# Sweetroll97/GaussianProcessPathModelling

Measured on AMD Instinct MI355X. Metric: gp_fit_predict_points_per_sec, higher is better.
Workload: dtype f64; 1 GPU; C3: exact GP fit+predict, N=65536 d=3 rbf float64, M=4096, inputs resident in HBM; N=65536, d=3, M=4096, kernel=rbf, block=2048, parallelism=1 gpu

## Files before the change

gaussianprocesspathmodelling_amd/csrc/gpx_api.hip:

```cpp
#include <hip/hip_runtime.h>
#include <dlfcn.h>

#include <algorithm>
#include <climits>
#include <cmath>
#include <cstdio>
#include <cstdlib>
#include <cstring>
#include <functional>
#include <new>
#include <string>
#include <vector>

#include "../../include/gpx.h"
#include "gpx_cov.h"
#include "gpx_env.h"
#include "gpx_internal.h"

using namespace gpx;

namespace {

thread_local std::string g_create_error;

// ... 150 lines not shown
}

bool bad_mem_kind(int32_t mem_kind) { return !(mem_kind == GPX_MEM_HOST || mem_kind == GPX_MEM_DEVICE); }

int fetch_ids(gpx_handle* h, const int32_t* src, int64_t n, int32_t mem_kind, std::vector<int32_t>& out) {
  out.resize((size_t)n);
  if (mem_kind == GPX_MEM_HOST) {
    std::copy(src, src + n, out.begin());
    return GPX_OK;
  }
  if (!h->group) HIPCHK(h, hipSetDevice(h->cfg.device));
  HIPCHK(h, hipMemcpy(out.data(), src, (size_t)n * sizeof(int32_t), hipMemcpyDefault));
  return GPX_OK;
}

int64_t first_below_minus_one(const int32_t* ids, int64_t n) {
  return std::find_if(ids, ids + n, [](int32_t v) { return v < -1; }) - ids;
}

bool variance_ok(double v) { return v >= 0.0 && std::isfinite(v); }
bool path_ls_ok(const double* ls_path, int32_t n) {
  return std::all_of(ls_path, ls_path + n, [](double l) { return l > 0.0 && std::isfinite(l); });
}

#define MATERN12_NO_GRAD "Matern-1/2 is not differentiable (its sample paths have no derivative)"
#define NOT_TWICE_DIFFERENTIABLE \
  "the kernel is not twice differentiable (only RBF and Matern-5/2 sample paths have a second derivative)"
#define HESS_D_LIMIT "second derivatives are built for at most 8 input dimensions (d > 8)"

#define LAUNCHCHK(h)                                                                                  \
  do {                                                                                                \
    if (take_launch_error())                                                                          \
      return fail(h, GPX_E_ARG, "internal error: a triangular-solve operand was not 128-byte aligned"); \
  } while (0)

int ensure(gpx_handle* h, DevBuf& b, size_t bytes) {
  if (b.cap >= bytes && b.p) return GPX_OK;
  if (b.p) HIPCHK(h, hipFree(b.p));
  b.p = nullptr;
  b.cap = 0;
  HIPCHK(h, hipMalloc(&b.p, bytes));
  b.cap = bytes;
  return GPX_OK;
}

hipEvent_t next_event(gpx_handle* h) {
  if (h->ev_used == h->ev_pool.size()) {
    hipEvent_t e;
    if (hipEventCreate(&e) != hipSuccess) return nullptr;
    h->ev_pool.push_back(e);
  }
  return h->ev_pool[h->ev_used++];
}

int record_event(gpx_handle* h, hipStream_t a, const char* site, hipEvent_t* e) {
  if (!(*e = next_event(h))) {
    char msg[64];
    snprintf(msg, sizeof msg, "hipEventCreate failed (%s)", site);
    return fail(h, GPX_E_HIP, msg);
  }
  HIPCHK(h, hipEventRecord(*e, a));
  return GPX_OK;
}

int stream_waits(gpx_handle* h, hipStream_t b, hipStream_t a, const char* site) {
  hipEvent_t e;
  if (int rc = record_event(h, a, site, &e)) return rc;
  HIPCHK(h, hipStreamWaitEvent(b, e, 0));
  return GPX_OK;
}

struct Roctx {
  int (*push)(const char*) = nullptr;
  int (*pop)() = nullptr;
};
const Roctx& roctx() {
  static const Roctx r = [] {
    Roctx x;
    EnvKnobs env;
    env_read(env, EnvAt::process);
    if (!env.roctx) return x;
    void* lib = nullptr;
    for (const char* n : {"librocprofiler-sdk-roctx.so.1", "librocprofiler-sdk-roctx.so", "libroctx64.so.4", "libroctx64.so"})
      if ((lib = dlopen(n, RTLD_NOW | RTLD_NOLOAD))) break;
    if (!lib)
      for (const char* n : {"librocprofiler-sdk-roctx.so.1", "librocprofiler-sdk-roctx.so"})
        if ((lib = dlopen(n, RTLD_NOW | RTLD_LOCAL))) break;
    if (!lib) return x;
    x.push = reinterpret_cast<int (*)(const char*)>(dlsym(lib, "roctxRangePushA"));
    x.pop = reinterpret_cast<int (*)()>(dlsym(lib, "roctxRangePop"));
    if (!x.push || !x.pop) x.push = nullptr, x.pop = nullptr;
    return x;
  }();
  return r;
}

const char* phase_name(const gpx_handle* h, const double* t) {
  const gpx_timings& tm = h->tm;
#define GPX_PHASE(f) \
  if (t == &tm.f) return "gpx:" #f;
  GPX_PHASE(h2d) GPX_PHASE(kbuild) GPX_PHASE(chol) GPX_PHASE(solve) GPX_PHASE(logdet) GPX_PHASE(fit_total)
  GPX_PHASE(kstar) GPX_PHASE(mean) GPX_PHASE(trsm) GPX_PHASE(var) GPX_PHASE(d2h) GPX_PHASE(predict_total)
  GPX_PHASE(comm) GPX_PHASE(chol_diag) GPX_PHASE(chol_trsm) GPX_PHASE(chol_strip) GPX_PHASE(chol_syrk)
  GPX_PHASE(grad_trtri) GPX_PHASE(grad_trace) GPX_PHASE(grad_total) GPX_PHASE(refine)
#undef GPX_PHASE
  return "gpx:phase";
}

struct PhaseScope {
  gpx_handle* h;
  Phase ph;
  bool on;
  hipStream_t s;
  bool ranged = false;
  PhaseScope(gpx_handle* h_, double* target, bool enable = true, hipStream_t stream = nullptr)
      : h(h_), on(enable), s(stream ? stream : h_->st) {
    if (roctx().push) ranged = roctx().push(phase_name(h, target)) >= 0;
    if (!on) return;
    ph.a = next_event(h);
    ph.b = next_event(h);
    ph.target = target;
    if (ph.a) (void)hipEventRecord(ph.a, s);
  }
  ~PhaseScope() {
    if (ranged) (void)roctx().pop();
    if (!on) return;
    if (ph.b) (void)hipEventRecord(ph.b, s);
    if (ph.a && ph.b) h->phases.push_back(ph);
  }
};

void collect_phases(gpx_handle* h) {
  for (auto& p : h->phases) {
    float ms = 0.f;
    if (hipEventElapsedTime(&ms, p.a, p.b) == hipSuccess) *p.target += ms;
  }
  h->phases.clear();
  h->ev_used = 0;
}


int flag_handover_probe(gpx_handle* h) {
  if (h->flag_ok >= 0) return GPX_OK;
  if (h->env.chain_flag >= 0) return GPX_OK;
  if (h->env.counters_collected || !h->st3) {
    h->flag_ok = 0;
    return GPX_OK;
  }
  unsigned* d = nullptr;
  unsigned seen = 0;
  HIPCHK(h, hipMalloc(&d, 64));
  hipError_t e = hipMemsetAsync(d, 0, 64, h->st);
  if (e == hipSuccess) e = hipStreamSynchronize(h->st);
  if (e == hipSuccess) {
    launch_flag_probe_wait(d, d + 1, 1u << 15, h->st3);
    launch_flag_probe_set(d, h->st);
    e = hipStreamSynchronize(h->st3);
  }
  if (e == hipSuccess) e = hipStreamSynchronize(h->st);
  if (e == hipSuccess) e = hipMemcpy(&seen, d + 1, sizeof(unsigned), hipMemcpyDeviceToHost);
  (void)hipFree(d);
  HIPCHK(h, e);
  h->flag_ok = seen ? 1 : 0;
  return GPX_OK;
}

bool chain_flag_enabled(const gpx_handle* h) {
  if (h->env.chain_flag >= 0) return h->env.chain_flag != 0;
  return !h->env.counters_collected && h->flag_ok == 1;
}

bool fused_strip_in_force(const gpx_handle* h) { return h->env.fused_strip && chain_flag_enabled(h); }
bool split_strip_in_force(const gpx_handle* h) { return h->env.split_strip && !fused_strip_in_force(h); }

bool retry_with_events(gpx_handle* h, bool retried) {
  if (retried || h->env.chain_flag >= 0) return false;
  h->flag_ok = 0;
  h->flag_retries += 1;
  return true;
}

struct LatencyGuard {
  ~LatencyGuard() { set_latency_mode(0); }
};
struct ReserveGuard {
  ~ReserveGuard() { reserve_ring(nullptr, 0); }
};
constexpr int RESV_RING = 1024;


template <typename T>
struct InvWork {
  T* W = nullptr;
  T* U = nullptr;
  int64_t ldu = 0;
  int nbw = 0;
  hipStream_t aux = nullptr;
  hipEvent_t ready = nullptr;
  hipEvent_t copied[2] = {};
  unsigned seq = 0;
};

template <typename T>
int diag_enqueue(gpx_handle* h, T* A, int64_t ld, int64_t o, int nbp, T* Winv, int* info, int64_t gidx0,
                 hipStream_t s, InvWork<T>* iw = nullptr) {
  T* Wp = nullptr;
  unsigned* dflag = reinterpret_cast<unsigned*>(info + 9);
  unsigned seq = iw ? iw->seq : 0;
  const bool use_flag = chain_flag_enabled(h);
  if (iw) {
    Wp = iw->W + (o / iw->nbw) * (int64_t)iw->nbw * iw->nbw;
    hipEvent_t e0 = next_event(h);
    if (!e0) return fail(h, GPX_E_HIP, "hipEventCreate failed (block inverse)");
    if (seq == 0) HIPCHK(h, hipMemsetAsync(dflag, 0, sizeof(unsigned), s));
    HIPCHK(h, hipEventRecord(e0, s));
    HIPCHK(h, hipStreamWaitEvent(iw->aux, e0, 0));
    HIPCHK(h, hipMemsetAsync(iw->U, 0, (size_t)iw->nbw * iw->ldu * sizeof(T), iw->aux));
    launch_set_diag_one_t<T>(iw->U, iw->ldu, nbp, iw->aux);
    HIPCHK(h, hipMemsetAsync(Wp, 0, (size_t)iw->nbw * iw->nbw * sizeof(T), iw->aux));
  }
  const int diag_step = h->env.diag_step;
  const int nq = nbp / KB;
  for (int q = 0; q < nq;) {
    const int w = (diag_step == 128 && q + 1 < nq) ? 2 : 1;
    const int64_t oq = o + (int64_t)q * KB;
    T* Aqq = A + oq * ld + oq;
    T* Wq = Winv + (oq / KB) * (KB * KB);
    seq += 2;
    if (w == 2)
      launch_potf2_128<T>(Aqq, ld, Wq, gidx0 + oq, info, s, iw && use_flag ? dflag : nullptr, seq);
    else
      launch_potf2_64<T>(Aqq, ld, Wq, gidx0 + oq, info, s, iw && use_flag ? dflag : nullptr, seq);
    const int64_t rem = o + nbp - (oq + w * KB);
    if (rem > 0) {
      T* panel = A + (oq + w * KB) * ld + oq;
      launch_trsm_rlt<T>(panel, ld, rem, Aqq, ld, Wq, w * KB, nullptr, 0, s);
      launch_gemm_nt<T>(64, A + (oq + w * KB) * ld + (oq + w * KB), ld, panel, ld, panel, ld, rem, rem, w * KB, 1, 0, s);
    }
    if (iw) {
      if (use_flag) {
        if (q > 0) {
          launch_wait_counter(dflag, seq - 1, info, iw->aux);
          launch_inv_extend<T>(iw->U, iw->ldu, A + o * ld + o, ld, Winv + (o / KB) * (KB * KB), q, q + w, Wp,
                               iw->nbw, iw->aux, 1);
        }
        launch_wait_counter(dflag, seq, info, iw->aux);
      } else {
        if (int rc = stream_waits(h, iw->aux, s, "block inverse")) return rc;
        launch_inv_extend<T>(iw->U, iw->ldu, A + o * ld + o, ld, Winv + (o / KB) * (KB * KB), q, q + w, Wp, iw->nbw,
                             iw->aux, 1);
      }
      launch_inv_extend<T>(iw->U, iw->ldu, A + o * ld + o, ld, Winv + (o / KB) * (KB * KB), q, q + w, Wp, iw->nbw,
                           iw->aux, 2);
    }
    q += w;
  }
  if (iw) {
    iw->seq = seq;
    if (int rc = record_event(h, iw->aux, "block inverse", &iw->ready)) return rc;
  }
  return GPX_OK;
}

template <typename T>
int panel_solve_enqueue(gpx_handle* h, T* A, int64_t ld, int64_t o, int nbp, int64_t rows_main, int64_t nx,
                        const T* Winv, T* P, int64_t ldp, hipStream_t s, InvWork<T>* iw, int set, int64_t row0 = 0,
                        hipEvent_t prev = nullptr, bool last = true) {
  T* Apanel = A + (o + nbp + row0) * ld + o;
  P += row0 * ldp;
  const int64_t rows = rows_main + nx;
  if (rows <= 0) {
    if (iw && last && row0 > 0) {
      if (int rc = record_event(h, h->st4, "panel copy", &iw->copied[set])) return rc;
    }
    return GPX_OK;
  }
  if (!iw) {
    launch_trsm_rlt<T>(Apanel, ld, rows, A + o * ld + o, ld, Winv + (o / KB) * (KB * KB), nbp, P, ldp, s);
    return GPX_OK;
  }
  const T* Wp = iw->W + (o / iw->nbw) * (int64_t)iw->nbw * iw->nbw;
  HIPCHK(h, hipStreamWaitEvent(s, iw->ready, 0));
  if (row0 == 0 && last) prev = iw->copied[set];
  if (prev) HIPCHK(h, hipStreamWaitEvent(s, prev, 0));
  const int tile_main = gemm_nt_tile((rows_main % 128 == 0 && nbp % 128 == 0) ? 128 : 64, rows_main, nbp, 4);
  if (rows_main > 0 && nx > 0 && tile_main == 64) {
    launch_gemm_nt_fixed<T>(64, P, ldp, Apanel, ld, Wp, iw->nbw, rows, nbp, nbp, 4, 1, s);
  } else {
    if (rows_main > 0) launch_gemm_nt_fixed<T>(tile_main, P, ldp, Apanel, ld, Wp, iw->nbw, rows_main, nbp, nbp, 4, 1, s);
    if (nx > 0)
      launch_gemm_nt<T>(64, P + rows_main * ldp, ldp, Apanel + rows_main * ld, ld, Wp, iw->nbw, nx, nbp, nbp, 4, 1,
                        s);
  }
  if (int rc = stream_waits(h, h->st4, s, "panel copy")) return rc;
  launch_copy2d<T>(Apanel, ld, P, ldp, rows, nbp, h->st4);
  if (last) return record_event(h, h->st4, "panel copy", &iw->copied[set]);
  return GPX_OK;
}

inline int64_t split_rows_128(int64_t nr, int64_t nc) {
  return (nr > 128 && nr % 128 != 0 && nc % 128 == 0) ? nr / 128 * 128 : nr;
}

template <typename T>
int chol_enqueue(gpx_handle* h, T* A, int64_t ld, int64_t n, int nb, T* Winv, T* P0, T* P1,
                 int64_t ldp, int* info, int64_t gidx0, bool profile, int64_t nx = 0,
                 InvWork<T>* iw = nullptr, int64_t nx_side = 0, int rest_split_arg = -1) {
  hipStream_t s0 = h->st, s1 = h->st2;
  T* Pbuf[2] = {P0, P1};
  int rc;
  const EnvKnobs& env = h->env;
  const bool fuse_env = fused_strip_in_force(h);
  unsigned* ctr = reinterpret_cast<unsigned*>(info + 8);
  unsigned target = 0;
  auto is_fused = [&](int64_t o) -> bool {
    if (!fuse_env || o >= n) return false;
    const int nbp = (int)std::min<int64_t>(nb, n - o);
    const int64_t ntrail = n - (o + nbp);
    if (ntrail <= 0) return false;
    const int nbn = (int)std::min<int64_t>(nb, ntrail);
    const int64_t nrest = ntrail - nbn;
    if (nrest <= 0 || ntrail % 128 != 0 || nbn % 128 != 0) return false;
    return gemm_nt_tile(128, nrest, nrest, 1) == 128 && gemm_nt_tile(128, ntrail, nbn, 2) == 128;
  };
  auto bordered_update = [&](int64_t o, const T* Pc, hipStream_t s) {
    const int nbp = (int)std::min<int64_t>(nb, n - o);
    const int64_t t0 = o + nbp, ntrail = n - t0;
    if (nx <= 0 || ntrail <= 0) return;
    launch_gemm_nt<T>(nx % 128 == 0 && ntrail % 128 == 0 ? 128 : 64, A + n * ld + t0, ld, Pc + ntrail * ldp, ldp, Pc,
                      ldp, nx, ntrail, nbp, 0, 0, s);
  };
  auto bordered_block = [&](int64_t o, const T* Pc, hipStream_t s, int64_t c0, int64_t nc, int64_t r0, int64_t nr) {
    const int nbp = (int)std::min<int64_t>(nb, n - o);
    const int64_t t0 = o + nbp, ntrail = n - t0;
    if (nr <= 0 || nc <= 0) return;
    const int64_t na = split_rows_128(nr, nc);
    launch_gemm_nt<T>(na % 128 == 0 && nc % 128 == 0 ? 128 : 64, A + (n + r0) * ld + c0, ld, Pc + (ntrail + r0) * ldp, ldp,
                      Pc + (c0 - t0) * ldp, ldp, na, nc, nbp, 0, 0, s);
    if (na < nr)
      launch_gemm_nt<T>(64, A + (n + r0 + na) * ld + c0, ld, Pc + (ntrail + r0 + na) * ldp, ldp, Pc + (c0 - t0) * ldp, ldp,
                        nr - na, nc, nbp, 0, 0, s);
  };
  auto update_is_big = [&](int64_t o) -> bool {
    if (o >= n) return false;
    const int nbp = (int)std::min<int64_t>(nb, n - o);
    const int64_t ntrail = n - (o + nbp);
    if (ntrail <= 0) return false;
    const int nbn = (int)std::min<int64_t>(nb, ntrail);
    const int64_t nrest = ntrail - nbn;
    return nrest > 0 && ntrail % 128 == 0 && nbn % 128 == 0 && gemm_nt_tile(128, nrest, nrest, 1) == 128;
  };
  const bool split_env = split_strip_in_force(h);
  const bool top_env = env.solve_top;
  const int rest_split = rest_split_arg >= 0 ? rest_split_arg : env.rest_split;
  const int64_t nxs = split_env ? nx_side : 0, nxc = nx - nxs;
  auto side_solve = [&](int64_t o, T* Pp, hipStream_t s) -> int {
    if (nxs <= 0) return GPX_OK;
    const int nbp = (int)std::min<int64_t>(nb, n - o);
    T* Aside = A + (n + nxc) * ld + o;
    T* Pside = Pp + ((n - o - nbp) + nxc) * ldp;
    if (!iw) {
      launch_trsm_rlt<T>(Aside, ld, nxs, A + o * ld + o, ld, Winv + (o / KB) * (KB * KB), nbp, Pside, ldp, s);
      return GPX_OK;
    }
    HIPCHK(h, hipStreamWaitEvent(s, iw->ready, 0));
    const T* Wp = iw->W + (o / iw->nbw) * (int64_t)iw->nbw * iw->nbw;
    const int64_t na = split_rows_128(nxs, nbp);
    launch_gemm_nt<T>(na % 128 == 0 && nbp % 128 == 0 ? 128 : 64, Pside, ldp, Aside, ld, Wp, iw->nbw, na, nbp, nbp, 4, 1, s);
    if (na < nxs) launch_gemm_nt<T>(64, Pside + na * ldp, ldp, Aside + na * ld, ld, Wp, iw->nbw, nxs - na, nbp, nbp, 4, 1, s);
    launch_copy2d<T>(Aside, ld, Pside, ldp, nxs, nbp, s);
    return GPX_OK;
  };
  LatencyGuard latency_guard;
  set_latency_mode(1);
  const int resv_k = env.cu_self_reserve;
  ReserveGuard reserve_guard;
  if (resv_k > 0 && split_env) {
    if ((rc = ensure(h, h->resv_ring, (size_t)RESV_RING * 8 * sizeof(unsigned)))) return rc;
    HIPCHK(h, hipMemsetAsync(h->resv_ring.p, 0, (size_t)RESV_RING * 8 * sizeof(unsigned), s0));
    reserve_ring((unsigned*)h->resv_ring.p, RESV_RING, env.resv_form);
  }
  const bool any_fused = is_fused(0);
  if (any_fused) HIPCHK(h, hipMemsetAsync(ctr, 0, sizeof(unsigned), s0));
  {
    const int nb0 = (int)std::min<int64_t>(nb, n);
    {
      PhaseScope ps(h, &h->tm.chol_diag, profile);
      if ((rc = diag_enqueue(h, A, ld, 0, nb0, Winv, info, gidx0, s0, iw))) return rc;
    }
    {
      PhaseScope ps(h, &h->tm.chol_trsm, profile);
      if ((rc = panel_solve_enqueue(h, A, ld, 0, nb0, n - nb0, nxc, Winv, Pbuf[0], ldp, s0, iw, 0))) return rc;
    }
    if (any_fused) {
      bordered_update(0, Pbuf[0], s0);
      if ((rc = stream_waits(h, s1, s0, "look-ahead"))) return rc;
    }
  }
  hipEvent_t e_main = nullptr;
  if (split_env && n > nb && (rc = record_event(h, s0, "look-ahead", &e_main))) return rc;
  int step = 0;
  for (int64_t o = 0; o < n; o += nb, ++step) {
    const int nbp = (int)std::min<int64_t>(nb, n - o);
    const int64_t t0 = o + nbp;
    const int64_t ntrail = n - t0;
    if (ntrail <= 0) {
      if ((rc = side_solve(o, Pbuf[step & 1], s0))) return rc;
      break;
    }
    T* Pc = Pbuf[step & 1];
    T* Pn = Pbuf[(step + 1) & 1];
    const int nbn = (int)std::min<int64_t>(nb, ntrail);
    const int64_t nrest = ntrail - nbn;
    const int tile = (ntrail % 128 == 0 && nbn % 128 == 0) ? 128 : 64;
    hipEvent_t e_panel = next_event(h);
    if (!e_panel) return fail(h, GPX_E_HIP, "hipEventCreate failed (look-ahead)");
    set_latency_mode(update_is_big(o) ? 0 : 1);
    if (is_fused(o)) {
      {
        PhaseScope ps(h, &h->tm.chol_syrk, profile);
        target += launch_gemm_nt_fused<T>(A + t0 * ld + t0, ld, Pc, ldp, ntrail, nbn, nbp, ctr, s0);
        h->tm.syrk_flops += (double)ntrail * (double)(ntrail + 1) * (double)nbp;
        h->tm.syrk_launches += 1;
      }
      launch_wait_counter(ctr, target, info, s1);
      {
        PhaseScope ps(h, &h->tm.chol_diag, profile, s1);
        if ((rc = diag_enqueue(h, A, ld, t0, nbn, Winv, info, gidx0, s1, iw))) return rc;
      }
      {
        PhaseScope ps(h, &h->tm.chol_trsm, profile, s1);
        if ((rc = panel_solve_enqueue(h, A, ld, t0, nbn, nrest, nx, Winv, Pn, ldp, s1, iw, (step + 1) & 1))) return rc;
      }
      HIPCHK(h, hipEventRecord(e_panel, s1));
      if (is_fused(t0)) bordered_update(t0, Pn, s1);
      HIPCHK(h, hipStreamWaitEvent(s0, e_panel, 0));
      continue;
    }
    if (split_env) {
      hipStream_t sm = s0;
      const int resv_it = (resv_k > 0 && (env.resv_all || ntrail <= (int64_t)(rest_split + 1) * nb)) ? resv_k : 0;
      if (e_main) HIPCHK(h, hipStreamWaitEvent(s1, e_main, 0));
      {
        PhaseScope ps(h, &h->tm.chol_strip, profile, s1);
        launch_gemm_nt<T>(tile, A + t0 * ld + t0, ld, Pc, ldp, Pc, ldp, nbn, nbn, nbp, 1, 0, s1);
      }
      set_reserve_mode(resv_it);
      {
        PhaseScope ps(h, &h->tm.chol_strip, profile, sm);
        if (nrest > 0)
          launch_gemm_nt<T>(tile, A + (t0 + nbn) * ld + t0, ld, Pc + (int64_t)nbn * ldp, ldp, Pc, ldp, nrest, nbn, nbp, 0,
                            0, sm);
        bordered_block(o, Pc, sm, t0, nbn, 0, nxc);
      }
      hipEvent_t e_below;
      if ((rc = record_event(h, sm, "look-ahead", &e_below))) return rc;
      const int nbn2 = (int)std::min<int64_t>(nb, nrest);
      const bool ahead = nrest > nbn2 && nrest <= (int64_t)rest_split * nb;
      T* Cr = A + (t0 + nbn) * ld + (t0 + nbn);
      const T* Pr = Pc + (int64_t)nbn * ldp;
      if (ahead) {
        {
          PhaseScope ps(h, &h->tm.chol_strip, profile, sm);
          launch_gemm_nt<T>(tile, Cr, ld, Pr, ldp, Pr, ldp, nrest, nbn2, nbp, 2, 0, sm);
        }
        if ((rc = record_event(h, sm, "look-ahead", &e_main))) return rc;
      }
      const int64_t nr = ahead ? nrest - nbn2 : nrest, off = ahead ? nbn2 : 0;
      if (nr > 0) {
        const bool big = gemm_nt_tile(tile, nr, nr, 1) == 128;
        PhaseScope ps(h, big ? &h->tm.chol_syrk : &h->tm.chol_strip, profile, sm);
        launch_gemm_nt<T>(tile, Cr + off * ld + off, ld, Pr + off * ldp, ldp, Pr + off * ldp, ldp, nr, nr, nbp, 1, 0, sm);
        if (big) {
          h->tm.syrk_flops += (double)nr * (double)(nr + 1) * (double)nbp;
          h->tm.syrk_launches += 1;
        }
      }
      if (!ahead && (rc = record_event(h, sm, "look-ahead", &e_main))) return rc;
      {
        PhaseScope ps(h, &h->tm.chol_strip, profile, sm);
        bordered_block(o, Pc, sm, t0 + nbn, nrest, 0, nxc);
        if ((rc = side_solve(o, Pc, sm))) return rc;
        bordered_block(o, Pc, sm, t0, ntrail, nxc, nxs);
      }
      set_reserve_mode(0);
      {
        PhaseScope ps(h, &h->tm.chol_diag, profile, s1);
        set_reserve_chain(resv_it > 0 ? env.resv_chain : 0);
        rc = diag_enqueue(h, A, ld, t0, nbn, Winv, info, gidx0, s1, iw);
        set_reserve_chain(0);
        if (rc) return rc;
      }
      HIPCHK(h, hipStreamWaitEvent(s1, e_below, 0));
      const int64_t top = (iw && top_env) ? std::min<int64_t>(nrest, nb) : nrest;
      hipEvent_t prev_copied = iw ? iw->copied[(step + 1) & 1] : nullptr;
      {
        PhaseScope ps(h, &h->tm.chol_trsm, profile, s1);
        if (top < nrest || (iw && top_env)) {
          if ((rc = panel_solve_enqueue(h, A, ld, t0, nbn, top, 0, Winv, Pn, ldp, s1, iw, (step + 1) & 1, 0, prev_copied,
                                        false)))
            return rc;
        } else if ((rc = panel_solve_enqueue(h, A, ld, t0, nbn, nrest, nxc, Winv, Pn, ldp, s1, iw, (step + 1) & 1))) {
          return rc;
        }
      }
      HIPCHK(h, hipEventRecord(e_panel, s1));
      HIPCHK(h, hipStreamWaitEvent(sm, e_panel, 0));
      if (top < nrest || (iw && top_env)) {
        PhaseScope ps(h, &h->tm.chol_trsm, profile, sm);
        set_reserve_mode(resv_it);
        rc = panel_solve_enqueue(h, A, ld, t0, nbn, nrest - top, nxc, Winv, Pn, ldp, sm, iw, (step + 1) & 1, top, prev_copied,
                                 true);
        set_reserve_mode(0);
        if (rc) return rc;
      }
      continue;
    }
    {
      PhaseScope ps(h, &h->tm.chol_strip, profile);
      set_latency_mode(1);
      launch_gemm_nt<T>(tile, A + t0 * ld + t0, ld, Pc, ldp, Pc, ldp, ntrail, nbn, nbp, 2, 0, s0);
      set_latency_mode(update_is_big(o) ? 0 : 1);
      bordered_update(o, Pc, s0);
    }
    if ((rc = stream_waits(h, s1, s0, "look-ahead"))) return rc;
    {
      {
        PhaseScope ps(h, &h->tm.chol_diag, profile, s1);
        if ((rc = diag_enqueue(h, A, ld, t0, nbn, Winv, info, gidx0, s1, iw))) return rc;
      }
      {
        PhaseScope ps(h, &h->tm.chol_trsm, profile, s1);
        if ((rc = panel_solve_enqueue(h, A, ld, t0, nbn, nrest, nx, Winv, Pn, ldp, s1, iw, (step + 1) & 1))) return rc;
      }
    }
    HIPCHK(h, hipEventRecord(e_panel, s1));
    if (nrest > 0) {
      const bool big = gemm_nt_tile(tile, nrest, nrest, 1) == 128;
      PhaseScope ps(h, big ? &h->tm.chol_syrk : &h->tm.chol_strip, profile);
      launch_gemm_nt<T>(tile, A + (t0 + nbn) * ld + (t0 + nbn), ld, Pc + (int64_t)nbn * ldp, ldp,
                        Pc + (int64_t)nbn * ldp, ldp, nrest, nrest, nbp, 1, 0, s0);
      if (big) {
        h->tm.syrk_flops += (double)nrest * (double)(nrest + 1) * (double)nbp;
        h->tm.syrk_launches += 1;
      }
    }
    HIPCHK(h, hipStreamWaitEvent(s0, e_panel, 0));
  }
  if (iw) {
    for (hipStream_t sj : {iw->aux, h->st4})
      if ((rc = stream_waits(h, s0, sj, "join"))) return rc;
  }
  return GPX_OK;
}

template <typename T>
int chol_two_level_enqueue(gpx_handle* h, T* A, int64_t ld, int64_t n, int nb, T* Winv, T* P0, T* P1, int64_t ldp,
                           int* info, int64_t gidx0, bool profile, int64_t nx = 0, InvWork<T>* iw = nullptr,
                           int64_t nx_side = 0) {
  const EnvKnobs& env = h->env;
  const int64_t c = std::max<int64_t>(1, (n / 2 + nb / 2) / nb) * nb, np = n - c;
  const int64_t smin = env.strassen_min;
  const int depth = smin > 0 ? (env.strassen_diag ? 2 : 1) : 0;
  const int64_t hh = np / 2 / 128 * 128, ldt = c / 2 + ld_skew<T>();
  const bool fits = P1 > P0 && strassen_temp_elems(np - hh, hh, c, ld_skew<T>()) <= 2 * (size_t)(P1 - P0);
  const bool wanted = depth == 0 || (fits && (sizeof(T) == 8 || env.strassen_f32));
  if (env.two_level_from <= 0 || n < env.two_level_from || !iw || nx_side != 0 || np < 256 || n % 128 != 0 || nb % 128 != 0 ||
      (nx != 0 && nx != RHS_ROWS) || !wanted)
    return chol_enqueue<T>(h, A, ld, n, nb, Winv, P0, P1, ldp, info, gidx0, profile, nx, iw, nx_side);
  int rc;
  hipStream_t s0 = h->st, s1 = h->st2;
  T *TA = P0, *TB = nullptr;
  const int rs = env.rest_split / 2;
  if ((rc = chol_enqueue<T>(h, A, ld, c, nb, Winv, P0, P1, ldp, info, gidx0, profile, np + nx, iw, np + nx, rs))) return rc;
  T* A22 = A + c * ld + c;
  const T* L21 = A + c * ld;
  hipEvent_t e_rows = nullptr;
  if (nx > 0) {
    if ((rc = stream_waits(h, s1, s0, "deep update"))) return rc;
    PhaseScope ps(h, &h->tm.chol_strip, profile, s1);
    launch_gemm_nt<T>(64, A + n * ld + c, ld, A + n * ld, ld, L21, ld, nx, np, c, 0, 0, s1);
    if ((rc = record_event(h, s1, "deep update", &e_rows))) return rc;
  }
  {
    PhaseScope ps(h, &h->tm.chol_syrk, profile);
    std::function<void(int64_t, int64_t, int)> deep = [&](int64_t o, int64_t sz, int lv) {
      const int64_t s1z = sz / 2 / 128 * 128, s2z = sz - s1z;
      if (lv <= 0 || s1z < 256 || std::min(s1z, s2z) / 256 * 128 < smin) {
        launch_gemm_nt<T>(128, A22 + o * ld + o, ld, L21 + o * ld, ld, L21 + o * ld, ld, sz, sz, c, 1, 0, s0);
        h->tm.syrk_flops += (double)sz * (double)(sz + 1) * (double)c;
        h->tm.syrk_launches += 1;
        return;
      }
      deep(o, s1z, lv - 1);
      TB = TA + (s2z / 256 * 128) * ldt;
      h->tm.syrk_flops += strassen_nt<T>(A22 + (o + s1z) * ld + o, ld, L21 + (o + s1z) * ld, ld, L21 + o * ld, ld, s2z, s1z,
                                         c, TA, TB, ldt, s0);
      h->tm.syrk_launches += 7;
      deep(o + s1z, s2z, lv - 1);
    };
    deep(0, np, depth);
  }
  if (e_rows) HIPCHK(h, hipStreamWaitEvent(s0, e_rows, 0));
  InvWork<T> iw2;
  iw2.W = iw->W + (c / iw->nbw) * (int64_t)iw->nbw * iw->nbw;
  iw2.U = iw->U;
  iw2.ldu = iw->ldu;
  iw2.nbw = iw->nbw;
  iw2.aux = iw->aux;
  rc = chol_enqueue<T>(h, A22, ld, np, nb, Winv + (c / KB) * (KB * KB), P0, P0 + (np + nx) * ldp, ldp, info, gidx0 + c, profile,
                       nx, &iw2, 0, rs);
  iw->seq = iw2.seq;
  return rc;
}

template <typename T>
struct SolveWork {
  const T* W = nullptr;
  int nbw = 0;
  T *T0 = nullptr, *T1 = nullptr;
  int64_t ldt = 0;
};

template <typename T>
int solve_fwd_enqueue(gpx_handle* h, T* XT, int64_t rows, const T* L, int64_t ld, int64_t n, int nb,
                      const T* Winv, const SolveWork<T>* wb = nullptr) {
  hipStream_t s0 = h->st, s1 = h->st2;
  const int tile = (rows % 128 == 0) ? 128 : 64;
  LatencyGuard latency_guard;
  set_latency_mode(1);
  if (rows < 128 || !s1) {
    for (int64_t o = 0; o < n; o += nb) {
      const int nbp = (int)std::min<int64_t>(nb, n - o);
      launch_trsm_rlt<T>(XT + o, ld, rows, L + o * ld + o, ld, Winv + (o / KB) * (KB * KB), nbp, nullptr,
                         0, s0);
      const int64_t ntrail = n - (o + nbp);
      if (ntrail > 0)
        launch_gemm_nt<T>((ntrail % 128 == 0) ? tile : 64, XT + o + nbp, ld, XT + o, ld,
                          L + (o + nbp) * ld + o, ld, rows, ntrail, nbp, 0, 0, s0);
    }
    return GPX_OK;
  }
  const bool dense = wb && wb->nbw == nb && wb->T0 && h->st4;
  T* Ts[2] = {dense ? wb->T0 : nullptr, dense ? wb->T1 : nullptr};
  hipEvent_t e_copy[2] = {nullptr, nullptr};
  const int64_t ldt = dense ? wb->ldt : 0;
  auto block_solve = [&](int64_t o, int nbp, int set, hipStream_t s) -> int {
    if (!dense) {
      launch_trsm_rlt<T>(XT + o, ld, rows, L + o * ld + o, ld, Winv + (o / KB) * (KB * KB), nbp, nullptr, 0, s);
      return GPX_OK;
    }
    if (e_copy[set]) HIPCHK(h, hipStreamWaitEvent(s, e_copy[set], 0));
    launch_gemm_nt<T>((rows % 128 == 0 && nbp % 128 == 0) ? 128 : 64, Ts[set], ldt, XT + o, ld,
                      wb->W + (o / nb) * (int64_t)nb * nb, nb, rows, nbp, nbp, 4, 1, s);
    hipEvent_t e = next_event(h);
    e_copy[set] = next_event(h);
    if (!e || !e_copy[set]) return fail(h, GPX_E_HIP, "hipEventCreate failed (block solve)");
    HIPCHK(h, hipEventRecord(e, s));
    HIPCHK(h, hipStreamWaitEvent(h->st4, e, 0));
    launch_copy2d<T>(XT + o, ld, Ts[set], ldt, rows, nbp, h->st4);
    HIPCHK(h, hipEventRecord(e_copy[set], h->st4));
    return GPX_OK;
  };
  int rc;
  if ((rc = block_solve(0, (int)std::min<int64_t>(nb, n), 0, s0))) return rc;
  int step = 0;
  for (int64_t o = 0; o < n; o += nb, ++step) {
    const int nbp = (int)std::min<int64_t>(nb, n - o);
    const int64_t t0 = o + nbp, ntrail = n - t0;
    if (ntrail <= 0) break;
    const int nbn = (int)std::min<int64_t>(nb, ntrail);
    const int64_t nrest = ntrail - nbn;
    const int tl = (nbn % 128 == 0 && nrest % 128 == 0) ? tile : 64;
    const int cur = step & 1;
    const T* Ablk = dense ? Ts[cur] : XT + o;
    const int64_t lda = dense ? ldt : ld;
    set_latency_mode(1);
    launch_gemm_nt<T>(tl, XT + t0, ld, Ablk, lda, L + t0 * ld + o, ld, rows, nbn, nbp, 0, 0, s0);
    set_latency_mode(nrest > 0 && gemm_nt_tile(tl, rows, nrest, 0) == 128 ? 0 : 1);
    hipEvent_t e_strip = next_event(h), e_panel = next_event(h);
    if (!e_strip || !e_panel) return fail(h, GPX_E_HIP, "hipEventCreate failed (look-ahead)");
    HIPCHK(h, hipEventRecord(e_strip, s0));
    HIPCHK(h, hipStreamWaitEvent(s1, e_strip, 0));
    if ((rc = block_solve(t0, nbn, cur ^ 1, s1))) return rc;
    HIPCHK(h, hipEventRecord(e_panel, s1));
    if (nrest > 0)
      launch_gemm_nt<T>(tl, XT + t0 + nbn, ld, Ablk, lda, L + (t0 + nbn) * ld + o, ld, rows, nrest, nbp, 0, 0,
                        s0);
    HIPCHK(h, hipStreamWaitEvent(s0, e_panel, 0));
  }
  if (dense) {
    for (int set = 0; set < 2; ++set)
      if (e_copy[set]) HIPCHK(h, hipStreamWaitEvent(s0, e_copy[set], 0));
  }
  return GPX_OK;
}

template <typename T>
void solve_bwd_enqueue(gpx_handle* h, T* XT, int64_t rows, const T* L, int64_t ld, int64_t n, int nb,
                       const T* Winv) {
  hipStream_t st = h->st;
  int64_t last = ((n - 1) / nb) * nb;
  for (int64_t o = last; o >= 0; o -= nb) {
    const int nbp = (int)std::min<int64_t>(nb, n - o);
    launch_trsm_rln<T>(XT + o, ld, rows, L + o * ld + o, ld, Winv + (o / KB) * (KB * KB), nbp, st);
    if (o > 0) launch_gemm_nn<T>(XT, ld, XT + o, ld, L + o * ld, ld, rows, o, nbp, st);
  }
}

int copy_in(gpx_handle* h, void* dst, const void* src, size_t bytes, int mem_kind) {
  if (bytes == 0) return GPX_OK;
  const hipMemcpyKind kind = mem_kind == GPX_MEM_HOST ? hipMemcpyHostToDevice
                             : h->in_group            ? hipMemcpyDefault
                                                      : hipMemcpyDeviceToDevice;
  HIPCHK(h, hipMemcpyAsync(dst, src, bytes, kind, h->st));
  return GPX_OK;
}

int copy_out(gpx_handle* h, void* dst, const void* src, size_t bytes, int mem_kind) {
  if (bytes == 0) return GPX_OK;
  HIPCHK(h, hipMemcpyAsync(dst, src, bytes,
                           mem_kind == GPX_MEM_HOST ? hipMemcpyDeviceToHost : hipMemcpyDeviceToDevice,
                           h->st));
  return GPX_OK;
}

int64_t pred_batch_rows(gpx_handle* h, int64_t Mpad, size_t row_bytes, bool may_shrink) {
  int64_t cap = h->env.pred_batch;
  if (may_shrink) {
    size_t freeb = 0, totalb = 0;
    if (hipMemGetInfo(&freeb, &totalb) == hipSuccess) {
      const double avail = 0.8 * ((double)freeb + (double)h->scr.VT.cap);
      const int64_t fit = (int64_t)(avail / (double)row_bytes) / 128 * 128;
      cap = std::max<int64_t>(128, std::min(cap, fit));
    }
  }
  return std::min(cap, Mpad);
}

int auto_panel_width(const gpx_handle* h, int64_t Npad) {
  const int64_t from = h->env.nb_wide_from;
  return (from > 0 && Npad >= from) ? 2048 : 1024;
}


void refresh_env(gpx_handle* h) { env_read(h->env, EnvAt::call); }

int begin_call(gpx_handle* h) {
  refresh_env(h);
  HIPCHK(h, hipSetDevice(h->cfg.device));
  h->err.clear();
  h->phases.clear();
  h->ev_used = 0;
  return GPX_OK;
}

int begin_fit(gpx_handle* h) {
  const int rc = begin_call(h);
  if (rc == GPX_OK) {
    h->fitted = false;
    h->basis = h->bp = 0;
    h->pw = {};
  }
  return rc;
}

int finish_call(gpx_handle* h) {
  HIPCHK(h, hipStreamSynchronize(h->st));
  HIPCHK(h, hipGetLastError());
  LAUNCHCHK(h);
  collect_phases(h);
  return GPX_OK;
}

void reset_predict_clocks(gpx_timings& tm) { tm.kstar = tm.mean = tm.trsm = tm.var = tm.d2h = tm.predict_total = 0; }

#define BY_DTYPE(h, fn, ...) ((h)->cfg.dtype == GPX_F32 ? fn<float>(__VA_ARGS__) : fn<double>(__VA_ARGS__))

template <typename T>
int ensure_queries(gpx_handle* h, int64_t M) {
  int rc;
  if ((rc = ensure(h, h->scr.Q, (size_t)M * h->d * sizeof(T)))) return rc;
  return ensure(h, h->scr.Qs, (size_t)round_up(M, TILE) * h->d * sizeof(T));
}

template <typename T>
int upload_queries(gpx_handle* h, const void* Xq, int64_t M, int32_t mem_kind) {
  int rc;
  if ((rc = copy_in(h, h->scr.Q.p, Xq, (size_t)M * h->d * sizeof(T), mem_kind))) return rc;
  launch_scale_points<T>((const T*)h->scr.Q.p, M, round_up(M, TILE), h->d, (const double*)h->ls.p, h->n_ls, (T*)h->scr.Qs.p,
                         h->st);
  return GPX_OK;
}

int upload_query_ids(gpx_handle* h, const int32_t* gq, int64_t M, int32_t mem_kind) {
  const int64_t Mpad = round_up(M, TILE);
  int rc;
  if ((rc = ensure(h, h->scr.Qg, (size_t)Mpad * sizeof(int32_t)))) return rc;
  HIPCHK(h, hipMemsetAsync(h->scr.Qg.p, 0xFF, (size_t)Mpad * sizeof(int32_t), h->st));
  return copy_in(h, h->scr.Qg.p, gq, (size_t)M * sizeof(int32_t), mem_kind);
}

template <typename T>
int dense_solve_work(gpx_handle* h, DevBuf& buf, int64_t rows, SolveWork<T>* sw) {
  if (h->nbw != h->nb_pred || (h->comm && !h->repl)) return GPX_OK;
  int rc;
  sw->ldt = h->nbw + ld_skew<T>();
  if ((rc = ensure(h, buf, (size_t)2 * rows * sw->ldt * sizeof(T)))) return rc;
  sw->W = (const T*)h->Wblk.p;
  sw->nbw = h->nbw;
  sw->T0 = (T*)buf.p;
  sw->T1 = sw->T0 + rows * sw->ldt;
  return GPX_OK;
}

template <typename T>
void mean_product(gpx_handle* h, T* MT, int64_t ldm, const T* rhsT, const T* VT, int64_t cols, T* part, int64_t ldpart) {
  const int ksplit = splitk_splits(h->Npad);
  if (ksplit > 1)
    launch_gemm_nt_splitk<T>(MT, ldm, rhsT, h->ld, VT, h->ld, RHS_ROWS, cols, h->Npad, ksplit, part, ldpart, h->st);
  else
    launch_gemm_nt<T>(64, MT, ldm, rhsT, h->ld, VT, h->ld, RHS_ROWS, cols, h->Npad, 0, 1, h->st);
}

template <typename T>
int ensure_mean_partials(gpx_handle* h, DevBuf& part, int64_t ldpart) {
  const int ksplit = splitk_splits(h->Npad);
  return ksplit > 1 ? ensure(h, part, (size_t)ksplit * RHS_ROWS * ldpart * sizeof(T)) : GPX_OK;
}

template <typename T>
void bordered_mean_var(gpx_handle* h, const T* VT, int64_t rows, int64_t rows_pad, int64_t ldm, bool want_var) {
  {
    PhaseScope ps(h, &h->tm.mean);
    mean_product<T>(h, (T*)h->scr.MT.p, ldm, (const T*)h->zT, VT, rows_pad, (T*)h->scr.MTpart.p, ldm);
    launch_unpack_rhs<T>((const T*)h->scr.MT.p, ldm, rows, h->k, 1.0, (T*)h->meanout.p, h->st);
  }
  if (want_var) {
    PhaseScope ps(h, &h->tm.var);
    launch_var_rows<T>(VT, h->ld, rows, h->Npad, h->sf2, (T*)h->var.p, h->st);
  }
  if (h->bp) {
    PhaseScope ps(h, want_var ? &h->tm.var : &h->tm.mean);
    launch_basis_epilogue<T>((const double*)h->Bst.p, h->bp, h->k, h->d, (const T*)h->scr.MT.p, ldm, (const T*)h->scr.Q.p, rows,
                             (T*)h->meanout.p, want_var ? (T*)h->var.p : nullptr, nullptr, h->st);
  }
}

template <typename T>
int deliver_mean_var(gpx_handle* h, void* mean, void* var, int64_t M, int32_t mem_kind) {
  PhaseScope ps(h, &h->tm.d2h);
  int rc;
  if ((rc = copy_out(h, mean, h->meanout.p, (size_t)M * h->k * sizeof(T), mem_kind))) return rc;
  return var ? copy_out(h, var, h->var.p, (size_t)M * sizeof(T), mem_kind) : GPX_OK;
}

template <typename T>
int predict_core(gpx_handle* h, const void* Xq, int64_t M, bool want_var, int32_t mem_kind, const int32_t* gq = nullptr);
bool few_solver_applies(const gpx_handle* h);
template <typename T>
int solve_few(gpx_handle* h, T* RT, int k, const T* L, int64_t ld, int64_t n, const T* W, int nb, bool forward = true,
              bool backward = true);

}

#include "gpx_shard.inc"
#include "gpx_group.inc"

namespace {

template <typename T>
int stage_fit_weights(gpx_handle* h, int64_t N, int64_t cap) {
  h->weighted = false;
  if (h->nw_set == 0) return GPX_OK;
  int rc;
  if ((rc = ensure(h, h->Wfit, (size_t)cap * sizeof(T)))) return rc;
  if (h->cfg.dtype == GPX_MIXED) {
// ... 3313 lines not shown
```

gaussianprocesspathmodelling_amd/csrc/gpx_env.h:

```cpp
#ifndef GPX_ENV_H_
#define GPX_ENV_H_

#include <cstdint>
#include <cstdio>
#include <cstdlib>
#include <cstring>

namespace gpx {

enum class EnvAt { create, call, process };

namespace env_rule {
inline bool flag(const char* e) { return atoi(e) != 0; }
inline int block(const char* e, int hi, int otherwise) {
  const int v = atoi(e);
  return (v >= 128 && v <= hi && v % 128 == 0) ? v : otherwise;
}
inline int64_t in_range(int64_t v, int64_t lo, int64_t hi, int64_t otherwise) { return (v >= lo && v <= hi) ? v : otherwise; }
}

#define GPX_ENV_TABLE(X)                                                                                               \
                                                               \
  X("GPX_DIAG_STEP", diag_step, Int, call, 128, atoi(e) == 64 ? 64 : 128)                                              \
  X("GPX_CHAIN_FLAG", chain_flag, Opt, call, -1, env_rule::flag(e))                                                    \
  X("GPX_FUSED_STRIP", fused_strip, Flag, call, false, env_rule::flag(e))                                              \
  X("GPX_SPLIT_STRIP", split_strip, Flag, call, true, env_rule::flag(e))                                               \
  X("GPX_SOLVE_TOP", solve_top, Flag, call, true, env_rule::flag(e))                                                   \
  X("GPX_REST_SPLIT", rest_split, Int, call, 16, atoi(e))                                                              \
  X("GPX_CU_SELF_RESERVE", cu_self_reserve, Int, call, 0, (int)env_rule::in_range(atoi(e), 1, 4, 0))                   \
  X("GPX_RESV_ALL", resv_all, Flag, call, false, env_rule::flag(e))                                                    \
  X("GPX_RESV_CHAIN", resv_chain, Int, call, 1, atoi(e))                                                               \
  X("GPX_RESV_FORM", resv_form, Int, call, 1, atoi(e))                                                                 \
                             \
  X("GPX_TWO_LEVEL_FROM", two_level_from, I64, call, 65536, env_rule::in_range(atoll(e), 0, 1L << 40, 0))                  \
  X("GPX_STRASSEN_MIN", strassen_min, I64, call, 4096, env_rule::in_range(atoll(e), 0, 1L << 40, 0) / 128 * 128)          \
  X("GPX_STRASSEN_DIAG", strassen_diag, Flag, call, false, env_rule::flag(e))                                          \
  X("GPX_STRASSEN_SINGLE", strassen_f32, Flag, call, false, env_rule::flag(e))                                            \
                                                                                            \
  X("GPX_NB_WIDE_FROM", nb_wide_from, I64, call, 40960, (int64_t)atoll(e))                                             \
  X("GPX_NB_GRAD", nb_grad, Int, call, 0, env_rule::block(e, 4096, 0))                                                 \
  X("GPX_NB_SOLVE", nb_solve, Int, create, 256, env_rule::block(e, 4096, 256))                                         \
  X("GPX_NB_PRED", nb_pred, Opt, create, -1, env_rule::block(e, 4096, 1024))                                           \
  X("GPX_NB_SHARD", nb_shard, Int, create, 0, env_rule::block(e, 2048, 0))                                             \
  X("GPX_PRED_BATCH", pred_batch, I64, call, 8192, env_rule::in_range(atol(e), 128, 1L << 22, 8192) / 128 * 128)       \
  X("GPX_FEW_SOLVE", few_solve, Flag, call, true, env_rule::flag(e))                                                   \
                                                                                         \
  X("GPX_SHARD_DEAL", shard_snake, Int, call, 1, (strcmp(e, "cyclic") == 0 || strcmp(e, "0") == 0) ? 0 : 1)            \
  X("GPX_SHARD_REPLICATE", shard_replicate, Opt, call, -1, env_rule::flag(e))                                          \
  X("GPX_SHARD_DENSE_PANEL", shard_dense_panel, Flag, call, true, env_rule::flag(e))                                   \
  X("GPX_SHARD_TWO_PIPE", shard_two_pipe, Opt, call, -1, env_rule::flag(e))                                            \
  X("GPX_SHARD_FUSED", shard_fused, Flag, call, true, env_rule::flag(e))                                               \
  X("GPX_REPL_COPY_SIDE", repl_copy_side, Flag, call, true, env_rule::flag(e))                                         \
  X("GPX_GROUP_INITALL", group_initall, Flag, call, true, env_rule::flag(e))                                           \
  X("GPX_LOCAL_FORCE_PEER", local_force_peer, Flag, call, false, env_rule::flag(e))                                    \
                                                                                                      \
  X("GPX_MICROBENCH_ITERS", microbench_iters, Int, call, 65536, (int)env_rule::in_range(atol(e), 64, 1L << 20, 65536)) \
  X("GPX_ROCTX", roctx, Flag, process, true, env_rule::flag(e))                                                        \
  X("GPX_RCCL_PATH", rccl_path, Str, process, nullptr, e)

struct EnvKnobs {
  using Flag = bool;
  using Int = int;
  using I64 = int64_t;
  using Opt = int;
  using Str = const char*;
#define GPX_ENV_FIELD(name, field, kind, at, dflt, rule) kind field = dflt;
  GPX_ENV_TABLE(GPX_ENV_FIELD)
#undef GPX_ENV_FIELD
  bool counters_collected = false;
};

inline void env_read(EnvKnobs& k, EnvAt at) {
#define GPX_ENV_READ(name, field, kind, at_, dflt, rule) \
  if (at == EnvAt::at_) {                                \
    const char* e = getenv(name);                        \
    k.field = e ? (rule) : (dflt);                       \
  }
  GPX_ENV_TABLE(GPX_ENV_READ)
#undef GPX_ENV_READ
  if (at == EnvAt::call) {
    const char* e = getenv("ROCPROF_COUNTER_COLLECTION");
    k.counters_collected = e && atoi(e) != 0;
  }
}

inline int env_print(const EnvKnobs& k, char* buf, int n) {
  int len = 0;
  auto put = [&](const char* name, const char* fmt, auto v) {
    const bool room = buf && n > 0 && len < n;
    const int w = snprintf(room ? buf + len : nullptr, room ? (size_t)(n - len) : 0, fmt, name, v);
    if (w > 0) len += w;
  };
  auto Flag = [&](const char* name, bool v) { put(name, "%s=%d\n", (int)v); };
  auto Int = [&](const char* name, int v) { put(name, "%s=%d\n", v); };
  auto I64 = [&](const char* name, int64_t v) { put(name, "%s=%lld\n", (long long)v); };
  auto Opt = [&](const char* name, int v) { v < 0 ? put(name, "%s=%s\n", "unset") : put(name, "%s=%d\n", v); };
  auto Str = [&](const char* name, const char* v) { put(name, "%s=%s\n", v ? v : "unset"); };
#define GPX_ENV_PRINT(name, field, kind, at, dflt, rule) kind(name, k.field);
  GPX_ENV_TABLE(GPX_ENV_PRINT)
#undef GPX_ENV_PRINT
  return len;
}

}

#endif
```

Baseline: 46020 points/s.

## Defer left-half side-block products into one Strassen GEMM during recursive Cholesky

In the recursive Cholesky path, the bordered side-block rows beyond the first half are no longer updated panel by panel. Their left-half contributions are accumulated as one large deferred GEMM, issued once the factor reaches the split column and run with Strassen when temp space allows. This replaces many thin panel GEMMs with one big product that can use the cheaper Strassen arithmetic. It adds event dependencies and extra complexity around the partial panel updates, and carries some numerical-accuracy risk from Strassen in f64. A new GPX_DEFER_LEFT env knob controls it, defaulting to on only for depth>0.

After: 46760 points/s, median of 6. +1.6%, better.

```diff
diff --git a/gaussianprocesspathmodelling_amd/csrc/gpx_api.hip b/gaussianprocesspathmodelling_amd/csrc/gpx_api.hip
--- a/gaussianprocesspathmodelling_amd/csrc/gpx_api.hip
+++ b/gaussianprocesspathmodelling_amd/csrc/gpx_api.hip
@@ -476,10 +476,17 @@
   return (nr > 128 && nr % 128 != 0 && nc % 128 == 0) ? nr / 128 * 128 : nr;
 }
 
+struct DeferLeft {
+  int64_t c1 = 0;
+  int64_t smin = 0;
+  size_t temp = 0;
+};
+
 template <typename T>
 int chol_enqueue(gpx_handle* h, T* A, int64_t ld, int64_t n, int nb, T* Winv, T* P0, T* P1,
                  int64_t ldp, int* info, int64_t gidx0, bool profile, int64_t nx = 0,
-                 InvWork<T>* iw = nullptr, int64_t nx_side = 0, int rest_split_arg = -1) {
+                 InvWork<T>* iw = nullptr, int64_t nx_side = 0, int rest_split_arg = -1,
+                 const DeferLeft* defer = nullptr) {
   hipStream_t s0 = h->st, s1 = h->st2;
   T* Pbuf[2] = {P0, P1};
   int rc;
@@ -545,6 +552,32 @@
     launch_copy2d<T>(Aside, ld, Pside, ldp, nxs, nbp, s);
     return GPX_OK;
   };
+  const int64_t dna0 = (defer && iw && nxs > 0 && !fuse_env && defer->c1 > 0 && defer->c1 < n && defer->c1 % nb == 0 && n % 128 == 0)
+                           ? split_rows_128(nxs, n - defer->c1)
+                           : 0;
+  const int64_t dna = dna0 % 128 == 0 ? dna0 : 0, dc1 = dna > 0 ? defer->c1 : 0;
+  auto deferred_product = [&](T* Tbuf, hipStream_t s) {
+    T* Cd = A + (n + nxc) * ld + dc1;
+    const T *Ad = A + (n + nxc) * ld, *Bd = A + dc1 * ld;
+    const int64_t nd = n - dc1, kd = dc1, ldt = kd / 2 + ld_skew<T>();
+    int64_t mch = 0;
+    for (int64_t parts = 1; defer->smin > 0 && parts <= dna / 256; ++parts) {
+      const int64_t m = round_up((dna + parts - 1) / parts, 256);
+      if (std::min(m, nd) / 256 * 128 < defer->smin) break;
+      if (strassen_temp_elems(m, nd, kd, ld_skew<T>()) <= defer->temp) {
+        mch = m;
+        break;
+      }
+    }
+    if (mch == 0) {
+      launch_gemm_nt<T>(128, Cd, ld, Ad, ld, Bd, ld, dna, nd, kd, 0, 0, s);
+      return;
+    }
+    for (int64_t r = 0; r < dna; r += mch) {
+      const int64_t m = std::min(mch, dna - r);
+      strassen_nt<T>(Cd + r * ld, ld, Ad + r * ld, ld, Bd, ld, m, nd, kd, Tbuf, Tbuf + (m / 256 * 128) * ldt, ldt, s);
+    }
+  };
   LatencyGuard latency_guard;
   set_latency_mode(1);
   const int resv_k = env.cu_self_reserve;
@@ -619,6 +652,8 @@
         PhaseScope ps(h, &h->tm.chol_strip, profile, s1);
         launch_gemm_nt<T>(tile, A + t0 * ld + t0, ld, Pc, ldp, Pc, ldp, nbn, nbn, nbp, 1, 0, s1);
       }
+      hipEvent_t e_stripd = nullptr;
+      if (t0 == dc1 && (rc = record_event(h, s1, "deferred product", &e_stripd))) return rc;
       set_reserve_mode(resv_it);
       {
         PhaseScope ps(h, &h->tm.chol_strip, profile, sm);
@@ -655,7 +690,19 @@
         PhaseScope ps(h, &h->tm.chol_strip, profile, sm);
         bordered_block(o, Pc, sm, t0 + nbn, nrest, 0, nxc);
         if ((rc = side_solve(o, Pc, sm))) return rc;
-        bordered_block(o, Pc, sm, t0, ntrail, nxc, nxs);
+        if (o < dc1) {
+          if (dc1 > t0)
+            launch_gemm_nt_fixed<T>(gemm_nt_tile(128, dna, ntrail, 0), A + (n + nxc) * ld + t0, ld, Pc + (ntrail + nxc) * ldp, ldp,
+                                    Pc, ldp, dna, dc1 - t0, nbp, 0, 0, sm);
+          bordered_block(o, Pc, sm, t0, ntrail, nxc + dna, nxs - dna);
+          if (t0 == dc1) {
+            if (iw->copied[step & 1]) HIPCHK(h, hipStreamWaitEvent(sm, iw->copied[step & 1], 0));
+            HIPCHK(h, hipStreamWaitEvent(sm, e_stripd, 0));
+            deferred_product(Pc, sm);
+          }
+        } else {
+          bordered_block(o, Pc, sm, t0, ntrail, nxc, nxs);
+        }
       }
       set_reserve_mode(0);
       {
@@ -746,7 +793,14 @@
   hipStream_t s0 = h->st, s1 = h->st2;
   T *TA = P0, *TB = nullptr;
   const int rs = env.rest_split / 2;
-  if ((rc = chol_enqueue<T>(h, A, ld, c, nb, Winv, P0, P1, ldp, info, gidx0, profile, np + nx, iw, np + nx, rs))) return rc;
+  DeferLeft defer;
+  defer.c1 = std::min<int64_t>(std::max<int64_t>(1, (c / 2 + nb / 2) / nb) * nb, c - nb);
+  defer.smin = depth > 0 ? smin : 0;
+  defer.temp = (size_t)(P1 - P0);
+  const bool defer_on = (env.defer_left < 0 ? depth > 0 : env.defer_left != 0) && defer.c1 > 0;
+  if ((rc = chol_enqueue<T>(h, A, ld, c, nb, Winv, P0, P1, ldp, info, gidx0, profile, np + nx, iw, np + nx, rs,
+                            defer_on ? &defer : nullptr)))
+    return rc;
   T* A22 = A + c * ld + c;
   const T* L21 = A + c * ld;
   hipEvent_t e_rows = nullptr;
diff --git a/gaussianprocesspathmodelling_amd/csrc/gpx_env.h b/gaussianprocesspathmodelling_amd/csrc/gpx_env.h
--- a/gaussianprocesspathmodelling_amd/csrc/gpx_env.h
+++ b/gaussianprocesspathmodelling_amd/csrc/gpx_env.h
@@ -36,6 +36,7 @@
   X("GPX_STRASSEN_MIN", strassen_min, I64, call, 4096, env_rule::in_range(atoll(e), 0, 1L << 40, 0) / 128 * 128)          \
   X("GPX_STRASSEN_DIAG", strassen_diag, Flag, call, false, env_rule::flag(e))                                          \
   X("GPX_STRASSEN_SINGLE", strassen_f32, Flag, call, false, env_rule::flag(e))                                            \
+  X("GPX_DEFER_LEFT", defer_left, Opt, call, -1, env_rule::flag(e))                                                    \
                                                                                             \
   X("GPX_NB_WIDE_FROM", nb_wide_from, I64, call, 40960, (int64_t)atoll(e))                                             \
   X("GPX_NB_GRAD", nb_grad, Int, call, 0, env_rule::block(e, 4096, 0))                                                 \
```
